# ybubnov/metalchat

Measured on AMD Instinct MI355X. Metric: decode tokens/s (batch=1) + achieved HBM GB/s vs roofline, int4 Llama-3-8B, higher is better.
Workload: dtype bf16

## Files before the change

metalchat_amd/csrc/decoder.cc:

```cpp

#include "decoder_impl.h"

using namespace mcimpl;

mc_decoder::~mc_decoder()
{
    (void)hipSetDevice(dev->ordinal);
    drop_graph();
    for (void* p : allocs) (void)hipFree(p);
    if (blas) blaslt_release(blas);
    if (err_evt) (void)hipEventDestroy(err_evt);
    if (err_host) (void)hipHostFree(err_host);
}

void
mc_decoder::query_occupancy()
{
    if (tb != 2 || occ_fused >= 0) return;
    auto ask = [&](const std::string& name, int block) {
        hipFunction_t f;
        if (fn(name, &f) != MC_OK) return 0;
        int n = 0;
        if (hipModuleOccupancyMaxActiveBlocksPerMultiprocessor(&n, f, block, 0) != hipSuccess) return 0;
        return n;
// ... 111 lines not shown
            P.chain_p = chain % 10;
            return one_launch(block_form::qkv_wo_w13_w, 1, vsh, "mc_attn_qkv_wo_w13_w_bfloat_hd64_k4_q4_f" + std::to_string(P.chain_f) + "p" + std::to_string(P.chain_p));
        }
        if (t) return one_launch(block_form::qkv_wo_w, t, vsh, std::string("mc_attn_qkv_wo_w_bfloat_hd64_k4_q4") + (t > 1 ? "_t" + std::to_string(t) : std::string()));
    }
    if (qkv_wo_in && opt.attn_i8_on && qkv.fmt == MC_WFMT_I8 && wo.fmt == MC_WFMT_I8 && occ_wo_i8 != 0) {
        auto group_ok = [](const linear_w& W) { return W.group == 0 || (W.group >= 16 && (W.group & (W.group - 1)) == 0); };
        const bool built = group_ok(qkv) && group_ok(wo) && qkv.group == wo.group && hd == 128 && wo.in == 4096 && qkv.in == 4096 && KV % 8 == 0 && n_rep <= 16;
        const int t = !built ? 0 : whole_range_tiles({1, 2, 4}, KV, [&](int, int ns, unsigned grid) {
            return deal_ok(pg, ns, 16) && (unsigned)wo.out / 2 <= 8u * grid;
        });
        if (t) return one_launch(block_form::qkv_wo_i8, t, 0, "mc_attn_qkv_wo_i8_bfloat_hd128_k4_q4_t" + std::to_string(t));
    }
    if (qkv_wo_in && i4_shape) {
        auto name = [&] { return "mc_attn_qkv_wo_i4_" + tname + "_hd128_k" + std::to_string(wo.in / 2048) + "_q" + std::to_string(qkv.in / 2048); };
        if (attn_wo_fused(wo) && deal_ok(pg, nsplit, 16) && pg >= 64 && pg <= 512) return one_launch(block_form::qkv_wo_i4, 1, 0, name());
        const int t = !opt.attn_i4_wide_on || occ_wo_i4_wide == 0 || KV % 8 != 0 ? 0 : whole_range_tiles({2, 4}, KV, [&](int, int ns, unsigned grid) {
            return deal_ok(pg, ns, 16) && pg >= 64 && (unsigned)wo.out / 2 <= 16u * grid;
        });
        if (t) return one_launch(block_form::qkv_wo_i4, t, 0, name() + "_t" + std::to_string(t));
    }
    if (!gemma && fused && opt.attn_qkv_on && opt.attn_qkv_only_on && occ_qkv_only != 0 && lin_ok(qkv) && !qkv.lora_cols && qkv_rows_ok && qkv.in == 8192 &&
        cfg.dim == 8192 && hd == 128 && KV % 8 == 0 && (unsigned)(nsplit * KV) <= (unsigned)dev->prop.multiProcessorCount && n_rep <= 16 && pg <= 1024 &&
        deal_ok(pg, nsplit, 24) && pg / nsplit >= 8) {
        P.wo_gemv = true;
        return one_launch(block_form::qkv_only, 1, 0, "mc_attn_qkv_i4_" + tname + "_hd128_q4");
    }
    int qkn_tiles = 0;
    if (gemma && handoffs_ok() && opt.attn_wo_qkn_on && opt.attn_wo_on && opt.attn_qkn_on && hd == 256 && occ_wo_qkn != 0 && lin_ok(wo) && !wo.lora_cols &&
        wo_rows_ok && wo.in == 4096 && n_rep <= 16)
        qkn_tiles = whole_range_tiles({1, 2, 4}, KV, [&](int t_, int, unsigned grid) {
// ... 16 lines not shown
        }
        one_launch(block_form::fused, 1, 0, "mc_attn_fused_" + tname);
        P.fast = handoff_mode_alone();
        P.grid = (unsigned)nsplit * ((P.fast & 2u) ? ((unsigned)KV + 7u) & ~7u : (unsigned)KV);
        return P;
    }
    if (attn_fused_t2()) {
        one_launch(block_form::fused_t2, 2, 0, "mc_attn_fused_t2_" + tname);
        P.fast = opt.handoff_fast ? 1u : 0u;
        return P;
    }
    P.form = block_form::scores_pv;
    P.name = "mc_attn_scores_" + tname;
    P.pv_fold = pv_fold(wo);
    return P;
}

mc_status
mc_decoder::check_handoffs(const step_state& st)
{
    if (!st.err) return MC_OK;
    return report_handoff(st.err);
}

mc_status
mc_decoder::report_handoff(uint32_t code)
{
    handoff_failed();
    char buf[384];
    snprintf(buf, sizeof buf, "decoder: an in-launch hand-off of the decode attention timed out (code 0x%08x): the workgroups of the "
// ... 354 lines not shown
    if (d->first_stage && !d->emb_table) return fail(MC_ERR_RUNTIME, "decoder: tok_embeddings not loaded");
    if (d->last_stage && (!d->output.allocated || !d->final_norm))
        return fail(MC_ERR_RUNTIME, "decoder: output head not loaded");
    if (d->cfg.family == MC_FAMILY_GEMMA3 && !d->pn_ready) {
        for (auto& L : d->layers) {
            if (!L.attention_post_norm || !L.ffn_post_norm) return fail(MC_ERR_RUNTIME, "decoder: post-norm weights are not loaded");
            const postnorm_args a{L.attention_post_norm, d->hidden, d->hidden_b};
            const postnorm_args f{L.ffn_post_norm, d->hidden_b, d->hidden};
            MC_HIP(hipMemcpy(L.pn_attn, &a, sizeof a, hipMemcpyHostToDevice));
            MC_HIP(hipMemcpy(L.pn_ffn, &f, sizeof f, hipMemcpyHostToDevice));
            d->pn_host[L.pn_attn] = a;
            d->pn_host[L.pn_ffn] = f;
        }
        d->pn_ready = true;
    }
    return MC_OK;
}

}

extern "C" {

mc_status
mc_decoder_create(mc_device* dev, mc_library* lib, mc_queue* q, const mc_decoder_config* cfg,
                  mc_decoder** out)
{
    if (!dev || !lib || !q || !cfg || !out)
        return fail(MC_ERR_INVALID_ARGUMENT, "mc_decoder_create: null argument");
    const mc_decoder_config& c = *cfg;
    if (c.n_heads % c.n_kv_heads != 0 || c.n_heads / c.n_kv_heads > 16)
// ... 677 lines not shown
```

metalchat_amd/csrc/decoder_impl.h:

```cpp
#pragma once

#include "backend_impl.h"
#include "decoder_batch.h"
#include "gemv_plan.h"

#include <algorithm>
#include <climits>
#include <cmath>
#include <cstddef>
#include <cstdio>
#include <cstdlib>
#include <cstring>
#include <initializer_list>
#include <map>
#include <memory>
#include <string>
#include <unordered_map>
#include <vector>

struct blaslt_state;

namespace mcimpl {

template <typename... A> inline void
push_all(arg_pack& p, const A&... a)
{
    (p.push(a), ...);
}

struct linear_w {
    int fmt = MC_WFMT_T;
    int out = 0, in = 0, group = 0;
    void* w = nullptr;
    void* scales = nullptr;
    size_t w_bytes = 0, s_bytes = 0;
    size_t row_bytes = 0;
    int ngroups = 1;
    bool allocated = false;
    std::vector<uint8_t> scales_host;
    void* wq2 = nullptr;
    uint64_t wq2_gen = 0;
    void* wd = nullptr;
    uint64_t wd_gen = 0;
    std::unique_ptr<linear_w> lora_a;
    void* lora_b = nullptr;
    std::vector<uint8_t> lora_b_host;
    void* lora_vec = nullptr;
    int lora_rank = 0;
    int lora_cols = 0;
    float lora_scale = 0.0f;
};

struct pick_block {
// ... 177 lines not shown
        return MC_OK;
    }
    float* rope_cos[2] = {nullptr, nullptr};
    float* rope_sin[2] = {nullptr, nullptr};
    int rope_rows = 0;
    int rope_start = 0;
    bool rope_valid = false;
    int last_pos = -1;
    bool want_taps = false;

    hipGraph_t graph = nullptr;
    hipGraphExec_t graph_exec = nullptr;

    std::vector<void*> allocs;
    bool pn_ready = false;
    bool log_on = false;
    std::vector<std::string> launch_log;

    ~mc_decoder();

    mc_status
    alloc(void** p, size_t bytes, bool zero = true)
    {
        hipError_t e = hipMalloc(p, bytes ? bytes : 16);
        if (e != hipSuccess)
            return fail(MC_ERR_ALLOC, std::string("hardware_memory_allocator: failed to allocate ") +
                                          std::to_string(bytes) + " bytes: " + hipGetErrorString(e));
        allocs.push_back(*p);
        if (zero) {
            MC_HIP(hipMemsetAsync(*p, 0, bytes ? bytes : 16, stream));
// ... 50 lines not shown
        void* extra[] = {HIP_LAUNCH_PARAM_BUFFER_POINTER, a.buf.data(), HIP_LAUNCH_PARAM_BUFFER_SIZE,
                         &n, HIP_LAUNCH_PARAM_END};
        mcimpl::launch_range range(name.c_str(), gx, gy, gz, bx, 1, 1);
        if (log_on) launch_log.push_back(name);
        hipError_t e = hipModuleLaunchKernel(f, gx, gy, gz, bx, 1, 1, lds, stream, nullptr, extra);
        if (e != hipSuccess) return hip_fail(e, name.c_str());
        return MC_OK;
    }

    size_t row_bytes(int fmt, int in) const;
    mc_status alloc_linear(linear_w& L, int fmt, int out, int in, int group);
    mc_status upload_rows(linear_w& L, int dst_row0, int dst_stride, int rows, const void* weight, const float* scales, int perm_hd = 0);

    gemv_env genv{};
    static gemv_shape
    shape_of(const linear_w& L) { return {L.fmt, L.out, L.in, L.group, L.lora_cols}; }
    bool
    lin_ok(const linear_w& L) const { return ::lin_ok(shape_of(L), genv); }
    bool
    lin_split_ok(const linear_w& L) const { return ::lin_split_ok(shape_of(L), genv); }
    int
    ling_kib(const linear_w& L) const { return ::ling_kib(shape_of(L), genv); }
    bool
    pv_fold(const linear_w& wo) const
    {
        return opt.pv_fold_on && (lin_ok(wo) || ling_kib(wo)) && !wo.lora_cols && cfg.max_seq_len <= 16384;
    }

    bool
    handoffs_ok() const { return attn_fused_on && attn_psum_g && tb == 2 && n_own <= 254; }
    unsigned
// ... 103 lines not shown
```

metalchat_amd/csrc/decoder_options.h:

```cpp
#pragma once

#include <algorithm>
#include <climits>
#include <cstdlib>

struct decoder_options {
    int gemv_block = 256;
    int gemv_wgs_per_cu = 2;
    bool gemv_block_env = false;
    bool gemv_lin = true;
    bool gemv_ling = true;
    bool i8_ling14 = true;
    bool lin_split = true;
    bool ling_half = true;
    bool lin_k4_on = true;
    int lin_waves = 8;
    bool gemv_full_grid = false;
    int dbg_variant = 0;
    int gemv_m4 = 2;
    int time_gemv_layers = 0;
    bool attn_fused = true;
    unsigned attn_fused_max_wgs_per_cu = 2;
    bool attn_t2_on = true;
    int rearm_after = 256;
    bool handoff_fast = true;
    bool attn_wo_on = true;
    bool attn_wo_k4 = false;
    bool attn_qkv_on = true;
    bool attn_qkv_only_on = false;
    bool attn_i8_on = true;
    bool attn_i4_wide_on = true;
    bool kv_virtual_on = true;
    bool chain_w13_on = true;
    int chain_f = -1;
    bool attn_qkv_qkn_on = true;
// ... 53 lines not shown
    o.gemv_wgs_per_cu = env_int("MC_GEMV_WGS_PER_CU", o.gemv_wgs_per_cu);
    o.gemv_block_env = env_set("MC_GEMV_BLOCK") || env_set("MC_GEMV_WGS_PER_CU");
    if (o.gemv_block % 64 || o.gemv_block < 64 || o.gemv_block > 1024) o.gemv_block = 256;
    if (o.gemv_wgs_per_cu < 1) o.gemv_wgs_per_cu = 2;
    o.gemv_lin = env_flag("MC_GEMV_LIN", o.gemv_lin);
    o.gemv_ling = env_flag("MC_GEMV_LING", o.gemv_ling);
    o.i8_ling14 = env_flag("MC_I8_LING14", o.i8_ling14);
    o.lin_split = env_flag("MC_LIN_SPLIT", o.lin_split);
    o.ling_half = env_flag("MC_LING_HALF", o.ling_half);
    o.lin_k4_on = env_flag("MC_LIN_K4", o.lin_k4_on);
    o.lin_waves = env_int("MC_LIN_WAVES", o.lin_waves, 1, 16);
    o.gemv_full_grid = env_flag("MC_GEMV_FULLGRID", o.gemv_full_grid);
    o.dbg_variant = env_int("MC_GEMV_DBG", o.dbg_variant);
    o.gemv_m4 = env_int("MC_GEMV_M4", o.gemv_m4);
    o.time_gemv_layers = env_int("MC_TIME_GEMV_LAYERS", 0, 0);

    o.attn_fused = env_flag("MC_ATTN_FUSED", o.attn_fused);
    o.attn_fused_max_wgs_per_cu = (unsigned)env_int("MC_ATTN_FUSED_WGS", (int)o.attn_fused_max_wgs_per_cu, 1, 4);
    o.attn_t2_on = env_flag("MC_ATTN_T2", o.attn_t2_on);
    o.rearm_after = env_int("MC_HANDOFF_REARM", o.rearm_after, 0);
    o.handoff_fast = env_flag("MC_HANDOFF_FAST", o.handoff_fast);
    o.attn_wo_on = env_flag("MC_ATTN_WO", o.attn_wo_on);
    o.attn_wo_k4 = env_set("MC_ATTN_WO_K4");
    o.attn_qkv_on = env_flag("MC_ATTN_QKV", o.attn_qkv_on);
    o.attn_qkv_only_on = env_flag("MC_ATTN_QKV_ONLY", o.attn_qkv_only_on);
    o.attn_i8_on = env_flag("MC_ATTN_I8", o.attn_i8_on);
    o.attn_i4_wide_on = env_flag("MC_ATTN_I4_WIDE", o.attn_i4_wide_on);
    o.kv_virtual_on = env_flag("MC_KV_VIRTUAL", o.kv_virtual_on);
    o.chain_w13_on = env_flag("MC_CHAIN_W13", o.chain_w13_on);
    o.chain_f = env_int("MC_CHAIN_F", o.chain_f, 0);
// ... 48 lines not shown
```

metalchat_amd/csrc/gemv_plan.h:

```cpp
#pragma once

#include <algorithm>
#include <cstdint>
#include <string>

#include "../../include/metalchat_hip.h"
#include "decoder_options.h"

struct gemv_shape {
    int fmt, out, in, group, lora_cols;
};
struct gemv_env {
    int tb;
    int qmode;
    unsigned cus;
    unsigned pick_slots;
    const decoder_options* opt;
};
enum class gemv_family { classic, fast, m4, m4d, lin, lin_k4, lin_split, ling };
struct gemv_plan {
    gemv_family family = gemv_family::classic;
    int rows_kib = 0;
    std::string name;
    unsigned wgs = 1, block = 256, lds = 0;
    bool postnorm_by_value = false;
    const char* error = nullptr;
};

inline size_t
gemv_row_bytes(int fmt, int in, int tb)
{
    if (fmt == MC_WFMT_I4) return (size_t)in / 2;
    if (fmt == MC_WFMT_I8) return (size_t)in;
    return (size_t)in * tb;
}
inline bool
gemv_i4_mfma(const gemv_shape& L, const gemv_env& e)
{
    return L.fmt == MC_WFMT_I4 && e.tb == 2 && e.qmode == MC_QMODE_EXACT && e.opt->gemv_m4 && !e.opt->dbg_variant;
// ... 37 lines not shown
}

inline unsigned
gemv_lin_cap(const gemv_env& e)
{
    return e.cus * (e.opt->gemv_block_env ? (unsigned)e.opt->gemv_wgs_per_cu : 1u);
}
inline unsigned
gemv_grid_per_cu(unsigned units, const gemv_env& e, unsigned at_least = 0)
{
    const unsigned waves = (unsigned)e.opt->lin_waves, cap = gemv_lin_cap(e);
    unsigned wgs = std::max((units + waves - 1) / waves, at_least);
    if (wgs > cap) wgs = cap;
    if (wgs > e.cus) wgs = wgs / e.cus * e.cus;
    return wgs;
}

inline gemv_plan
plan_gemv(const gemv_shape& L, const gemv_env& e, int pro, int epi)
{
    const decoder_options& opt = *e.opt;
    const unsigned cus = e.cus;
    gemv_plan P;
    const int nch = gemv_nch(L);
    const bool lin = lin_ok(L, e) && !(pro == 2 && L.lora_cols);
    const int pe_code = pro * 10 + epi;
    const bool lins = !lin && lin_split_ok(L, e) &&
                      (pe_code == 0 || pe_code == 10 || pe_code == 1 || pe_code == 12 || pe_code == 13 || pe_code == 14 || pe_code == 20 || pe_code == 23);
    const int ling = lin || lins || pro == 2 ? 0 : ling_kib(L, e);
    if (pro == 3 && !lin && !ling) {
// ... 14 lines not shown
             : ling ? gemv_family::ling
             : gemv_i4_mfma(L, e) ? (m4d ? gemv_family::m4d : gemv_family::m4)
             : fast ? gemv_family::fast : gemv_family::classic;
    P.rows_kib = lin ? nch : ling;
    P.postnorm_by_value = pro == 2 && (lin || lins);

    const unsigned kpl = L.fmt == MC_WFMT_I4 ? 32 : (L.fmt == MC_WFMT_I8 ? 16 : (e.tb == 2 ? 8 : 4));
    const unsigned chunk = 64 * kpl;
    const unsigned row = (unsigned)((size_t)((L.in + chunk - 1) / chunk) * chunk * e.tb);
    const unsigned lin_block = 64u * (unsigned)opt.lin_waves, parked = (unsigned)opt.lin_waves * 512u;
    const unsigned np = (unsigned)L.out / 2;
    std::string suffix;
    switch (P.family) {
    case gemv_family::lin:
    case gemv_family::lin_k4:
        suffix = "_lin" + std::to_string(nch) + (k4 ? "k4" : "");
        P.wgs = k4 ? cus : gemv_grid_per_cu(np, e);
        P.block = lin_block;
        P.lds = row / 16 * 17 + 128 + parked;
        break;
    case gemv_family::lin_split:
        suffix = "_lin3s";
        P.wgs = gemv_grid_per_cu((unsigned)L.out / 4, e);
        P.block = lin_block;
        P.lds = 3u * chunk * (unsigned)e.tb / 16 * 17 + 128 + parked;
        break;
    case gemv_family::ling: {
        suffix = "_ling" + std::to_string(ling);
        const unsigned waves = (unsigned)opt.lin_waves, cap = gemv_lin_cap(e);
        const bool half = opt.ling_half && (epi == 0 || epi == 1) && !L.lora_cols && 2u * np <= cap * waves && (unsigned)L.out % 2 == 0;
        P.wgs = gemv_grid_per_cu(np, e, half ? std::min(cap, ((unsigned)L.out + waves - 1) / waves) : 0u);
// ... 6 lines not shown
    case gemv_family::fast:
    case gemv_family::classic:
        suffix = P.family == gemv_family::m4d ? "_m4d" : P.family == gemv_family::m4 ? "_m4" : P.family == gemv_family::fast ? "_fast" : "";
        P.wgs = classic_wgs;
        P.block = classic_block;
        P.lds = (P.family == gemv_family::m4d ? row / 16 * 17 : row) + 128;
        break;
    }
    if (L.fmt == MC_WFMT_I4 && e.tb == 2 && opt.dbg_variant && ((pro == 1 && epi == 2) || (pro == 0 && epi == 0)))
        suffix += opt.dbg_variant == 1 ? "_dbgstream" : "_dbgnoload";
    P.name = std::string("mc_gemv_") + (L.fmt == MC_WFMT_I4 ? "i4_" : (L.fmt == MC_WFMT_I8 ? "i8_" : "w_")) + (e.tb == 2 ? "bfloat" : "float") + suffix +
             "_p" + std::to_string(pro) + "_e" + std::to_string(epi);
    if (epi == 5 && P.wgs > e.pick_slots) P.wgs = e.pick_slots;
    return P;
}
```

metalchat_amd/csrc/kernels/attn_block_kernels.hip:

```cpp
#include "gemv.h"

namespace {

using namespace mc;
using namespace mc::gemv;


#ifndef MC_QKV_ROW_DEAL
#define MC_QKV_ROW_DEAL 0
#endif
#ifndef MC_QX_STG_I4
#define MC_QX_STG_I4 1
#endif
#ifndef MC_QX_STG_I8
#define MC_QX_STG_I8 2
#endif
#ifndef MC_QX_STG_W
#define MC_QX_STG_W 0
#endif
template <int HD, int QN, int WB = 0, int STG = (WB == 0 ? MC_QX_STG_I4 : (WB == 1 ? MC_QX_STG_W : MC_QX_STG_I8))>
struct qkv_in_launch {
    static_assert(WB ? QN == 4 : (QN == 2 || QN == 4), "K = 4096 / 8192 int4, 4096 int8, 2048 bfloat; 512 threads");
    static constexpr bool WIDE = WB == 0 && QN == 4;
#ifndef MC_I8_SCORER_WAVES
#define MC_I8_SCORER_WAVES 8
#endif
    static constexpr int SCORER_WAVES = MC_I8_SCORER_WAVES;
    static constexpr bool LDS = true, PIN_V = true, STAGED = STG != 0;
    static constexpr int K_STEPS = WB == 1 ? 1 : (WIDE ? 3 : 2), V_STEP = STG == 2 ? K_STEPS : K_STEPS - 1;
    static constexpr int TL_STRIDE = 16, TL_BASE = 3;
    static constexpr uint32_t KQ = WB == 1 ? 512u * QN : (WB == 2 ? 1024u * QN : 2048u * QN), ROWBQ = 1024u * QN, CHUNK_LDS = 2048 * 2 / 16 * 17, HALF = HD / 2;
    static constexpr uint32_t NPK = KQ / 8;
    static constexpr uint32_t WPK = WB == 1 ? 8u : (WB == 2 ? 16u : 32u);
    static constexpr int PMAXQ = WB == 1 ? 1 : (WIDE ? 3 : 2);
    static constexpr int NXP = WIDE ? 2 : 1;
    typedef const __attribute__((address_space(3))) bf16_t* lds_row;
// ... 586 lines not shown
                    ((gS_p)vt)[((size_t)kv * HD + 2u * j) * max_seq + slot] = va;
                    ((gS_p)vt)[((size_t)kv * HD + 2u * j + 1u) * max_seq + slot] = vb;
                }
            }
        }
        lds_barrier();
        stamp(11);
    }
};

struct gemma_extra {
    const void *post_w, *res_row;
    void* h_out;
    const bf16_t *q_norm, *k_norm;
};
template <int HD, int LNCH, int QN = 0, int WB = 0, int TT = 1, int QKN = 0, int CH = 0>
__device__ __forceinline__ void
attn_wo_body(const bf16_t* __restrict__ q, const bf16_t* __restrict__ kc, const bf16_t* __restrict__ vt, bf16_t* __restrict__ attn_out,
             unsigned long long* psum_g, unsigned long long* slab_g, unsigned long long* row_g, step_state* st, uint32_t n_rep,
             uint32_t KV, uint32_t max_seq, float scale, uint32_t nsplit, uint32_t layer_tag, const void* __restrict__ wo_w,
             const void* __restrict__ wo_s, const bf16_t* res, bf16_t* y, uint32_t out_rows, uint32_t group, uint32_t has_res,
             uint32_t fastpath, unsigned long long* tl,
             const void* __restrict__ qnorm_w = nullptr, const void* __restrict__ qkv_w = nullptr, const void* __restrict__ qkv_s = nullptr,
             const float* fcos = nullptr, const float* fsin = nullptr, unsigned long long* qkv_g = nullptr, float eps = 0.0f, float mu = 0.0f,
             uint32_t kv_shift = 0, gemma_extra gx = gemma_extra(), unsigned long long* hid_g = nullptr)
{
    static_assert(CH == 0 || (QN != 0 && QKN == 0), "a chained phase: behind a llama launch with wq|wk|wv inside");
    constexpr uint32_t K = WB == 1 ? 512u * LNCH : (WB == 2 ? 1024u * LNCH : 2048u * LNCH);
    constexpr uint32_t WPK = WB == 1 ? 8u : (WB == 2 ? 16u : 32u);
    constexpr uint32_t CHUNK_LDS = 2048 * 2 / 16 * 17;
    constexpr uint32_t ROWB = 1024u * LNCH;
    constexpr int QCH = QKN >= 2 ? 3 : QN;
    __shared__ __attribute__((aligned(16))) char xs[(LNCH > QCH ? LNCH : QCH) * (WB == 1 ? 1024u : (WB == 2 ? 2048u : CHUNK_LDS))];
    static_assert(QN == 0 || QKN == 0, "one source of the step's queries");
    __shared__ float qred[(QN || QKN) ? 32 : 1];
    __shared__ __attribute__((aligned(16))) bf16_t qkv_rows[(QN || QKN) ? 18 * HD : 8];
    const uint32_t tid = threadIdx.x, lane = tid & 63, wave = __builtin_amdgcn_readfirstlane(tid >> 6);
    typedef qkv_in_launch<HD, QN ? QN : (WB ? 4 : 2), WB> qx_t;
    qx_t qx;
    if constexpr (QN != 0) {
        typedef typename qx_t::lds_row lds_row;
        qx.q_s = (lds_row)qkv_rows;
        qx.k_s = (lds_row)qkv_rows + n_rep * HD;
        qx.v_s = (lds_row)qkv_rows + (n_rep + 1u) * HD;
        qx.xp = res; qx.normp = qnorm_w; qx.qw = qkv_w; qx.qs = qkv_s; qx.fcos = fcos; qx.fsin = fsin;
        qx.kc = const_cast<bf16_t*>(kc); qx.vt = const_cast<bf16_t*>(vt); qx.qkv_g = qkv_g; qx.st = st; qx.xs = xs; qx.red = qred;
        qx.n_rep = n_rep; qx.KV = KV; qx.max_seq = max_seq; qx.nsplit = nsplit; qx.group = group; qx.layer_tag = layer_tag;
        qx.fastpath = fastpath; qx.eps = eps; qx.mu = mu; qx.tl = tl; qx.kv_shift = kv_shift;
        qx.at_start();
    }
    typedef qkv_qkn_in_launch<(QKN >= 2 ? HD : 256), QKN == 3> qg_t;
    qg_t qg;
    if constexpr (QKN >= 2) {
// ... 202 lines not shown
    stamp(7);
}

}

#define MC_ATTN_WO(NAME, HD, LNCH)                                                                                                        \
    extern "C" __global__ void __launch_bounds__(512)                                                                                    \
    NAME(const bf16_t* q, const bf16_t* kc, const bf16_t* vt, bf16_t* attn_out, unsigned long long* psum_g, unsigned long long* slab_g, \
         unsigned long long* row_g, step_state* st, uint32_t n_rep, uint32_t n_kv, uint32_t max_seq, float scale, uint32_t nsplit,      \
         uint32_t layer_tag, const void* wo_w, const void* wo_s, const bf16_t* res, bf16_t* y, uint32_t out_rows, uint32_t group,       \
         uint32_t has_res, uint32_t fastpath, unsigned long long* tl)                                                                    \
    {                                                                                                                                    \
        attn_wo_body<HD, LNCH>(q, kc, vt, attn_out, psum_g, slab_g, row_g, st, n_rep, n_kv, max_seq, scale, nsplit, layer_tag, wo_w,     \
                               wo_s, res, y, out_rows, group, has_res, fastpath, tl);                                                    \
    }
#define MC_ATTN_QKV_WO(NAME, HD, LNCH, QN, TT)                                                                                            \
    extern "C" __global__ void __launch_bounds__(512)                                                                                    \
    NAME(const bf16_t* kc, const bf16_t* vt, bf16_t* attn_out, unsigned long long* psum_g, unsigned long long* slab_g,                  \
         unsigned long long* row_g, unsigned long long* qkv_g, step_state* st, uint32_t n_rep, uint32_t n_kv, uint32_t max_seq,         \
         float scale, uint32_t nsplit, uint32_t layer_tag, const void* wo_w, const void* wo_s, const bf16_t* x, bf16_t* y,              \
         uint32_t out_rows, uint32_t group, const void* qnorm_w, const void* qkv_w, const void* qkv_s, const float* fcos, const float* fsin, float eps,    \
         float mu, uint32_t fastpath, unsigned long long* tl, uint32_t kv_shift)                                                         \
    {                                                                                                                                    \
        attn_wo_body<HD, LNCH, QN, 0, TT>(nullptr, kc, vt, attn_out, psum_g, slab_g, row_g, st, n_rep, n_kv, max_seq, scale, nsplit,     \
                                          layer_tag, wo_w, wo_s, x, y, out_rows, group, 1u, fastpath, tl, qnorm_w, qkv_w, qkv_s, fcos,   \
                                          fsin, qkv_g, eps, mu, kv_shift);                                                               \
    }
MC_ATTN_QKV_WO(mc_attn_qkv_wo_i4_bfloat_hd128_k2_q2, 128, 2, 2, 1)
MC_ATTN_QKV_WO(mc_attn_qkv_wo_i4_bfloat_hd128_k2_q2_t2, 128, 2, 2, 2)
MC_ATTN_QKV_WO(mc_attn_qkv_wo_i4_bfloat_hd128_k2_q2_t4, 128, 2, 2, 4)
template <int HD, int QN>
__device__ __forceinline__ void
attn_qkv_body(const bf16_t* kc, const bf16_t* vt, bf16_t* attn_out, unsigned long long* psum_g, unsigned long long* slab_g, unsigned long long* qkv_g,
              step_state* st, uint32_t n_rep, uint32_t KV, uint32_t max_seq, float scale, uint32_t nsplit, uint32_t layer_tag, const bf16_t* x,
              uint32_t group, const void* norm_w, const void* qkv_w, const void* qkv_s, const float* fcos, const float* fsin, float eps, float mu,
              uint32_t fastpath, unsigned long long* tl)
{
    constexpr uint32_t CHUNK_LDS = 2048 * 2 / 16 * 17;
    __shared__ __attribute__((aligned(16))) char xs[QN * CHUNK_LDS];
    __shared__ float qred[16];
    __shared__ __attribute__((aligned(16))) bf16_t qkv_rows[18 * HD];
    typedef qkv_in_launch<HD, QN, 0> qx_t;
    typedef typename qx_t::lds_row lds_row;
    qx_t qx;
    qx.q_s = (lds_row)qkv_rows;
// ... 267 lines not shown
```

metalchat_amd/csrc/kernels/decode_kernels.hip:

```cpp
#include "common.h"
#include "handoff.h"
#include <type_traits>

using namespace mc;


__device__ __forceinline__ void
derive_state(step_state* st, int32_t max_seq, int32_t pre_len)
{
    const int32_t post = max_seq - pre_len;
    if (st->pos >= max_seq) {
        st->ring_base = (st->ring_base + 1) % post;
        st->rolled += 1;
        st->write_slot = pre_len + (post - 1 + st->ring_base) % post;
        st->kv_len = max_seq;
    } else {
        const int32_t p = st->pos;
        st->write_slot = p < pre_len ? p : pre_len + (p - pre_len + st->ring_base) % post;
        st->kv_len = p + 1;
    }
    st->rope_row = st->pos - st->rope_start;
    st->epoch += 1;
}

// ... 602 lines not shown
        if (HPP < n_rep + 1u) one_pass(HPP, std::integral_constant<int, 1>{});
        if (2u * HPP < n_rep + 1u) one_pass(2u * HPP, std::integral_constant<int, 2>{});
        for (uint32_t h0 = 3u * HPP; h0 < n_rep + 1u; h0 += HPP) one_pass(h0, std::integral_constant<int, NPRE>{});
        for (uint32_t d = tid; d < (uint32_t)HD; d += NT) {
            const bf16_t v = qkv[(size_t)(H + KV + kv) * HD + d];
            ((lds_row_w)v_s)[d] = v;
            if (writer) vt[((size_t)kv * HD + d) * max_seq + ws] = v;
        }
        lds_barrier();
    }
};
template <typename Q, typename = void>
struct scorer_waves_of { static constexpr int value = 4; };
template <typename Q>
struct scorer_waves_of<Q, std::void_t<decltype(Q::SCORER_WAVES)>> { static constexpr int value = Q::SCORER_WAVES; };
template <int HD, int T, int NW, bool PADKV = false, typename OnChunk, typename BehindScores, typename QSrc = q_from_hbm>
__device__ __forceinline__ void
attn_fused_bf(const bf16_t* __restrict__ q, const bf16_t* __restrict__ kc, const bf16_t* __restrict__ vt,
              unsigned long long* psum_g, unsigned long long* slab_g, step_state* st, uint32_t n_rep, uint32_t KV, uint32_t max_seq,
              float scale, uint32_t nsplit, uint32_t layer_tag, unsigned long long* tl, OnChunk&& on_chunk, BehindScores&& behind_scores,
              uint32_t fastpath, QSrc qsrc = QSrc(), uint32_t kv_shift = 0)
{
    const size_t psum_fast = (size_t)KV * n_rep * nsplit, slab_fast = (size_t)KV * nsplit * n_rep * HD;
    auto stamp = [&](int i) {
        if (tl && threadIdx.x == 0) tl[(size_t)blockIdx.x * QSrc::TL_STRIDE + QSrc::TL_BASE + i] = __builtin_amdgcn_s_memrealtime();
    };
    stamp(0);
    constexpr int KS = HD / 32;
    constexpr int NDB = HD / 16;
    constexpr int NB = NDB >= NW ? NDB / NW : 1;
    constexpr uint32_t PBW = PB * T;
    constexpr int SW = (NW == 8 && T >= 2 && scorer_waves_of<QSrc>::value == 8) ? 8 : 4;
    constexpr int TS = T * 4 / SW;
    constexpr uint32_t PBS = 16u * SW;
    constexpr int ES = PBW + 4;
    __shared__ float wsum[SW][16];
    __shared__ float inv_s[16];
    __shared__ __attribute__((aligned(16))) float ebuf[16 * ES];

    const uint32_t kv_stride = (PADKV && (fastpath & 2u)) ? ((KV + 7u) & ~7u) : KV;
    const uint32_t kv = blockIdx.x % kv_stride, split = blockIdx.x / kv_stride;
    if constexpr (PADKV) {
        if (kv >= KV) return;
    }
    const uint32_t lane = threadIdx.x & 63, wave = threadIdx.x >> 6;
    const uint32_t col = lane & 15, c = lane >> 4;
    const uint32_t p_begin = split * PBW;
    const uint32_t kvc = kv >> kv_shift;
    qsrc.before_tiles();
    uint4 kb[TS][KS];
    const bool scorer = NW == 4 || wave < (uint32_t)SW;
    auto request_k_lds = [&](int t) {
        const size_t live = (size_t)0 - (size_t)(scorer ? 1 : 0);
        const uint32_t pos = p_begin + t * PBS + wave * 16 + col;
        const bf16_t* kbase = kc + ((((size_t)kvc * max_seq + (pos < max_seq ? pos : max_seq - 1)) * HD + c * 8) & live);
#pragma unroll
        for (int ks = 0; ks < KS; ks++) kb[t][ks] = *reinterpret_cast<const uint4*>(kbase + ks * 32);
    };
    if constexpr (QSrc::LDS) {
        if constexpr (!QSrc::STAGED) {
#pragma unroll
            for (int t = 0; t < TS; t++) request_k_lds(t);
        }
    } else if (scorer) {
#pragma unroll
        for (int t = 0; t < TS; t++) {
            const uint32_t pos = p_begin + t * PBS + wave * 16 + col;
            const bf16_t* kbase = kc + ((size_t)kvc * max_seq + (pos < max_seq ? pos : max_seq - 1)) * HD;
#pragma unroll
            for (int ks = 0; ks < KS; ks++) kb[t][ks] = *reinterpret_cast<const uint4*>(kbase + ks * 32 + c * 8);
        }
    }
    uint4 vb[T][NB][2];
    auto request_v = [&] {
#pragma unroll
        for (int t = 0; t < T; t++)
#pragma unroll
            for (int b = 0; b < NB; b++) {
                const uint32_t db = wave + NW * b;
                const bf16_t* vrow = vt + ((size_t)kvc * HD + (db < (uint32_t)NDB ? db : 0u) * 16 + col) * max_seq;
#pragma unroll
                for (int u = 0; u < 2; u++) {
                    const uint32_t p0 = p_begin + t * PB + u * 32 + c * 8;
                    vb[t][b][u] = *reinterpret_cast<const uint4*>(vrow + (p0 + 8 <= max_seq ? p0 : max_seq - 8));
                }
            }
    };
    constexpr bool V_LATE = QSrc::LDS && !QSrc::PIN_V;
    if constexpr (!V_LATE && !QSrc::STAGED) request_v();
    if constexpr (QSrc::LDS && QSrc::STAGED) {
        qsrc.before_scores([&](int step) {
            asm volatile("" ::: "memory");
#pragma unroll
            for (int t = 0; t < TS; t++)
                if (step == (t < QSrc::K_STEPS ? t : QSrc::K_STEPS - 1)) request_k_lds(t);
            if (step == QSrc::V_STEP && !V_LATE) request_v();
            asm volatile("" ::: "memory");
        });
        uint32_t never;
// ... 517 lines not shown
```

metalchat_amd/csrc/kernels/gemv.h:

```cpp
#pragma once
#ifndef MC_ABL_NORM_NOXWAVE
#define MC_ABL_NORM_NOXWAVE 0
#endif

#include "abi.h"
#include "common.h"

#include <type_traits>

namespace mc {
namespace gemv {

enum { WF_T = 0, WF_I8 = 1, WF_I4 = 2 };
enum { Q_EXACT = 0, Q_FAST = 1, Q_DBG_STREAM = 2, Q_DBG_NOLOAD = 3,
       Q_M4 = 5,
       Q_M4D = 6 };
enum { PRO_NONE = 0, PRO_RMSNORM = 1, PRO_POSTNORM = 2, PRO_PARTS = 3 };
constexpr int PARTS_R = 4;

static __device__ __forceinline__ void lds_barrier() { asm volatile("s_waitcnt lgkmcnt(0)\n\ts_barrier" ::: "memory"); }
using abi::postnorm_args;
enum { EPI_STORE = 0, EPI_RESID = 1, EPI_SILU_MUL = 2, EPI_GELU_MUL = 3, EPI_QKV_ROPE = 4, EPI_STORE_PICK = 5 };
using abi::pick_epilogue;
__device__ __forceinline__ unsigned long long
// ... 411 lines not shown
        auto cnt_a = [&](uint32_t i) { return e + sq + (i < sr ? 1u : 0u) + (i < ra ? 1u : 0u); };
        auto cnt_b = [&](uint32_t i) { return e - sq - (i < sr ? 1u : 0u) + (i < rb ? 1u : 0u); };
        const uint32_t a_all = 4u * (e + sq) + sr + ra;
        const uint32_t mine = wave < 4 ? cnt_a(w4) : cnt_b(w4);
        const uint32_t before = wave < 4 ? w4 * (e + sq) + min(w4, sr) + min(w4, ra) : a_all + w4 * (e - sq) - min(w4, sr) + min(w4, rb);
        pb = sb0 + before;
        pe = pb + mine;
    } else {
        const uint32_t nw_total = gridDim.x * nwaves, gw = blockIdx.x * nwaves + wave;
        const uint32_t pq = NP / nw_total, prem = NP - pq * nw_total;
        pb = gw * pq + min(gw, prem);
        pe = pb + pq + (gw < prem ? 1u : 0u);
    }
}

template <int WF, typename T, int QM, int PRO, int EPI, int R, int LNCH = 0, int LTP = 0, int LRING = 0, int LWAVES = 0, int LGEN = 0, int LSPLIT = 0>
__device__ __forceinline__ void
body(const void* __restrict__ wp, const void* __restrict__ sp, const void* __restrict__ xp,
     void* __restrict__ yp, const void* __restrict__ resp, const void* __restrict__ normp,
     uint32_t out_rows, uint32_t in, uint32_t group, float eps, float mu,
     const void* __restrict__ lora_ap, const void* __restrict__ lora_bp, uint32_t lora_rank,
     float lora_scale)
{
    using F = fmt<WF, T>;
    using S = typename T::S;
    constexpr int KPL = F::KPL;
    constexpr uint32_t CHUNK = 64 * KPL;
    constexpr uint32_t CHUNK_BYTES = 64 * 16;
    static_assert(R == 4, "tiles are four rows deep (scale quads, paired epilogues)");

    if (LNCH > 0 || LGEN > 0) {
// ... 696 lines not shown
        auto ltile = [&](uint4 (&dst)[LTP], uint32_t pr, int t, bool live) {
            const uint32_t chunk0 = (uint32_t)(t % SUB) * LTP;
            const uint64_t rb = ((uint64_t)pr * 2 + (uint64_t)(t / SUB)) * rowb_l + (uint64_t)chunk0 * 1024;
            const uint32_t lm = 0u - (uint32_t)live;
            const uint64_t lm64 = ((uint64_t)lm << 32) | lm;
            const char* a = wbase + (rb & lm64);
            const uint32_t lo = lane16 & lm;
#pragma unroll
            for (int p = 0; p < LTP; p++) {
                if (MC_GEMV_LIN_NOLOAD) {
                    dst[p] = make_uint4(lane * 0x01010101u + pr, (lane + pr) * 0x9E3779B9u, lane * 0x85EBCA6Bu + (uint32_t)(t * 0x11111111u),
                                        (p + lane) * 0xC2B2AE35u + pr);
                    continue;
                }
                const u32x4* ap = reinterpret_cast<const u32x4*>(a + p * 1024 + lo);
#ifndef MC_LIN_PLAIN_LOADS
#define MC_LIN_PLAIN_LOADS 0
#endif
                const u32x4 v = MC_LIN_PLAIN_LOADS ? *ap : __builtin_nontemporal_load(ap);
                dst[p] = make_uint4(v.x, v.y, v.z, v.w);
            }
        };
        auto lscales = [&](uint32_t (&q)[LNCH], uint32_t pr, bool live) {
            const uint64_t ub = (((uint64_t)(pr >> 1) * ngroups) * 4 + (pr & 1u) * 2) * 2;
            const uint32_t lm = 0u - (uint32_t)live;
            const char* a = sbase + (ub & (((uint64_t)lm << 32) | lm));
#pragma unroll
            for (int c = 0; c < LNCH; c++) {
                if (MC_GEMV_LIN_NOLOAD) {
                    q[c] = 0x3C003C00u;
                    continue;
                }
                const uint32_t g = group ? ((2048u * (uint32_t)c + 32u * lane) >> glog) : 0u;
                q[c] = *reinterpret_cast<const uint32_t*>(a + ((g * 8u) & lm));
// ... 356 lines not shown
```

metalchat_amd/csrc/kernels/gemv_kernels.hip:

```cpp
#include "gemv.h"
#include "gemv_ksplit.h"

using namespace mc;
using namespace mc::gemv;

#ifndef MC_GEMV_LB
#define MC_GEMV_LB 512
#endif
#define MC_GEMV(NAME, WF, T, QM, PRO, EPI)                                                        \
    extern "C" __global__ void __launch_bounds__(MC_GEMV_LB)                                          \
    NAME(const void* w, const void* scales, const void* x, void* y, const void* res,             \
         const void* norm_w, uint32_t out_rows, uint32_t in, uint32_t group, float eps, float mu, \
         const void* lora_a, const void* lora_b, uint32_t lora_rank, float lora_scale)            \
    {                                                                                             \
        body<WF, T, QM, PRO, EPI, 4>(w, scales, x, y, res, norm_w, out_rows, in, group, eps, mu,  \
                                     lora_a, lora_b, lora_rank, lora_scale);                      \
    }

#ifndef MC_LIN_WAVES
#define MC_LIN_WAVES 8
#endif
#define MC_GEMV_LIN(NAME, PRO, EPI, ...)                                                          \
    extern "C" __global__ void __launch_bounds__(MC_LIN_WAVES ? 64 * MC_LIN_WAVES : MC_GEMV_LB)   \
    NAME(const void* w, const void* scales, const void* x, void* y, const void* res,             \
// ... 56 lines not shown
#endif
#ifndef MC_LIN7_CFG
#define MC_LIN7_CFG 7, 1, 2
#endif
#ifndef MC_LIN12_CFG
#define MC_LIN12_CFG 12, 1, 2
#endif
#ifndef MC_LIN14_CFG
#define MC_LIN14_CFG 14, 1, 2
#endif
MC_GEMV_LIN_SET(mc_gemv_i4_bfloat_lin1, MC_LIN1_CFG)
MC_GEMV_LIN_SET(mc_gemv_i4_bfloat_lin2, MC_LIN2_CFG)
MC_GEMV_LIN_SET(mc_gemv_i4_bfloat_lin4, MC_LIN4_CFG)
MC_GEMV_LIN_SET(mc_gemv_i4_bfloat_lin7, MC_LIN7_CFG)
MC_GEMV_LIN_SET(mc_gemv_i4_bfloat_lin12, MC_LIN12_CFG)
#define MC_GEMV_K4(NAME, NCH, EPI)                                                                \
    extern "C" __global__ void __launch_bounds__(512)                                             \
    NAME(const void* w, const void* scales, const void* x, void* y, const void* res,             \
         const void* norm_w, uint32_t out_rows, uint32_t in, uint32_t group, float eps, float mu, \
         const void* lora_a, const void* lora_b, uint32_t lora_rank, float lora_scale)            \
    {                                                                                             \
        body_ksplit4<NCH, EPI>(w, scales, x, y, res, out_rows, group);                            \
    }
MC_GEMV_K4(mc_gemv_i4_bfloat_lin12k4_p0_e0, 12, 0)
MC_GEMV_K4(mc_gemv_i4_bfloat_lin12k4_p0_e1, 12, 1)
#ifndef MC_LIN3S_RING
#define MC_LIN3S_RING 3
#endif
#define MC_GEMV_LINS(NAME, PRO, EPI)                                                              \
    extern "C" __global__ void __launch_bounds__(64 * MC_LIN_WAVES)                               \
// ... 52 lines not shown
```

Measured before the change: 768.6.

## Plan cache-resident FFN weights and stream KV tiles with non-temporal loads

Adds a planner that picks per-layer w13/w2 weights to keep in the last-level cache, using plain loads through new resident GEMV kernel twins. All other weights keep non-temporal loads. It also adds a non-temporal variant of the fused int4 qkv/wo attention kernel for K/V tile loads, used for layers after the first when the streamed set exceeds the cache size. The aim is to stop streaming data from evicting reusable lines. It risks extra kernel variants, and the resident budget is off by default.

```diff
diff --git a/metalchat_amd/csrc/decoder.cc b/metalchat_amd/csrc/decoder.cc
--- a/metalchat_amd/csrc/decoder.cc
+++ b/metalchat_amd/csrc/decoder.cc
@@ -149,7 +149,8 @@
     }
     if (qkv_wo_in && i4_shape) {
         auto name = [&] { return "mc_attn_qkv_wo_i4_" + tname + "_hd128_k" + std::to_string(wo.in / 2048) + "_q" + std::to_string(qkv.in / 2048); };
-        if (attn_wo_fused(wo) && deal_ok(pg, nsplit, 16) && pg >= 64 && pg <= 512) return one_launch(block_form::qkv_wo_i4, 1, 0, name());
+        const bool nt = kv_nt && tname == "bfloat" && wo.in == 4096 && qkv.in == 4096 && !layers.empty() && &L != &layers[0];
+        if (attn_wo_fused(wo) && deal_ok(pg, nsplit, 16) && pg >= 64 && pg <= 512) return one_launch(block_form::qkv_wo_i4, 1, 0, name() + (nt ? "_nt" : ""));
         const int t = !opt.attn_i4_wide_on || occ_wo_i4_wide == 0 || KV % 8 != 0 ? 0 : whole_range_tiles({2, 4}, KV, [&](int, int ns, unsigned grid) {
             return deal_ok(pg, ns, 16) && pg >= 64 && (unsigned)wo.out / 2 <= 16u * grid;
         });
@@ -196,6 +197,34 @@
     P.name = "mc_attn_scores_" + tname;
     P.pv_fold = pv_fold(wo);
     return P;
+}
+
+void
+mc_decoder::plan_resident_set()
+{
+    resident_planned = true;
+    kv_nt = false;
+    for (layer_w& L : layers) L.w13.resident = L.w2.resident = false;
+    if (!first_stage || !last_stage || layers.empty()) return;
+    const bool gemma = cfg.family == MC_FAMILY_GEMMA3;
+    std::vector<resident_layer> sizes(layers.size());
+    size_t streamed = linear_bytes(output);
+    for (size_t li = 0; li < layers.size(); li++) {
+        layer_w& L = layers[li];
+        streamed += linear_bytes(L.qkv) + linear_bytes(L.wo) + linear_bytes(L.w13) + linear_bytes(L.w2);
+        streamed += 2 * (size_t)cfg.n_kv_heads * cfg.max_seq_len * cfg.head_dim * tb;
+        auto offer = [&](linear_w& W, int pro, int epi) -> size_t {
+            gemv_shape sh = shape_of(W);
+            sh.resident = true;
+            const gemv_plan P = plan_gemv(sh, genv, pro, epi);
+            return !P.error && P.resident ? linear_bytes(W) : (size_t)0;
+        };
+        sizes[li] = resident_layer{{0, 0, gemma ? 0 : offer(L.w13, 1, 2), gemma ? 0 : offer(L.w2, 0, 1)}};
+    }
+    static const std::vector<int> ranks[4] = {{RES_W2, RES_W13}, {RES_W13, RES_W2}, {RES_W2}, {RES_W13}};
+    const auto set = plan_resident(sizes, streamed, (size_t)opt.mall_resident_mb << 20, ranks[opt.mall_rank]);
+    for (const auto& p : set) (p.second == RES_W2 ? layers[p.first].w2 : layers[p.first].w13).resident = true;
+    kv_nt = opt.mall_kv_nt == 2 || (opt.mall_kv_nt == 1 && (streamed > MALL_BYTES || !set.empty()));
 }
 
 mc_status
@@ -580,6 +609,7 @@
         }
         d->pn_ready = true;
     }
+    if (!d->resident_planned) d->plan_resident_set();
     return MC_OK;
 }
 
diff --git a/metalchat_amd/csrc/decoder_impl.h b/metalchat_amd/csrc/decoder_impl.h
--- a/metalchat_amd/csrc/decoder_impl.h
+++ b/metalchat_amd/csrc/decoder_impl.h
@@ -37,6 +37,7 @@
     size_t row_bytes = 0;
     int ngroups = 1;
     bool allocated = false;
+    bool resident = false;
     std::vector<uint8_t> scales_host;
     void* wq2 = nullptr;
     uint64_t wq2_gen = 0;
@@ -244,6 +245,8 @@
 
     std::vector<void*> allocs;
     bool pn_ready = false;
+    bool resident_planned = false, kv_nt = false;
+    void plan_resident_set();
     bool log_on = false;
     std::vector<std::string> launch_log;
 
@@ -324,7 +327,7 @@
 
     gemv_env genv{};
     static gemv_shape
-    shape_of(const linear_w& L) { return {L.fmt, L.out, L.in, L.group, L.lora_cols}; }
+    shape_of(const linear_w& L) { return {L.fmt, L.out, L.in, L.group, L.lora_cols, L.resident}; }
     bool
     lin_ok(const linear_w& L) const { return ::lin_ok(shape_of(L), genv); }
     bool
diff --git a/metalchat_amd/csrc/decoder_options.h b/metalchat_amd/csrc/decoder_options.h
--- a/metalchat_amd/csrc/decoder_options.h
+++ b/metalchat_amd/csrc/decoder_options.h
@@ -19,6 +19,9 @@
     int dbg_variant = 0;
     int gemv_m4 = 2;
     int time_gemv_layers = 0;
+    int mall_resident_mb = 0;
+    int mall_kv_nt = 1;
+    int mall_rank = 0;
     bool attn_fused = true;
     unsigned attn_fused_max_wgs_per_cu = 2;
     bool attn_t2_on = true;
@@ -102,6 +105,9 @@
     o.dbg_variant = env_int("MC_GEMV_DBG", o.dbg_variant);
     o.gemv_m4 = env_int("MC_GEMV_M4", o.gemv_m4);
     o.time_gemv_layers = env_int("MC_TIME_GEMV_LAYERS", 0, 0);
+    o.mall_resident_mb = env_int("MC_MALL_RESIDENT_MB", o.mall_resident_mb, 0, 256);
+    o.mall_kv_nt = env_int("MC_MALL_KV_NT", o.mall_kv_nt, 0, 2);
+    o.mall_rank = env_int("MC_MALL_RANK", o.mall_rank, 0, 3);
 
     o.attn_fused = env_flag("MC_ATTN_FUSED", o.attn_fused);
     o.attn_fused_max_wgs_per_cu = (unsigned)env_int("MC_ATTN_FUSED_WGS", (int)o.attn_fused_max_wgs_per_cu, 1, 4);
diff --git a/metalchat_amd/csrc/gemv_plan.h b/metalchat_amd/csrc/gemv_plan.h
--- a/metalchat_amd/csrc/gemv_plan.h
+++ b/metalchat_amd/csrc/gemv_plan.h
@@ -3,12 +3,15 @@
 #include <algorithm>
 #include <cstdint>
 #include <string>
+#include <utility>
+#include <vector>
 
 #include "../../include/metalchat_hip.h"
 #include "decoder_options.h"
 
 struct gemv_shape {
     int fmt, out, in, group, lora_cols;
+    bool resident = false;
 };
 struct gemv_env {
     int tb;
@@ -23,6 +26,7 @@
     int rows_kib = 0;
     std::string name;
     unsigned wgs = 1, block = 256, lds = 0;
+    bool resident = false;
     bool postnorm_by_value = false;
     const char* error = nullptr;
 };
@@ -90,6 +94,12 @@
     if (wgs > cap) wgs = cap;
     if (wgs > e.cus) wgs = wgs / e.cus * e.cus;
     return wgs;
+}
+
+inline bool
+resident_twin(int nch, int pro, int epi)
+{
+    return (nch == 7 && pro == 0 && epi == 1) || (nch == 2 && pro == 1 && epi == 2);
 }
 
 inline gemv_plan
@@ -134,7 +144,8 @@
     switch (P.family) {
     case gemv_family::lin:
     case gemv_family::lin_k4:
-        suffix = "_lin" + std::to_string(nch) + (k4 ? "k4" : "");
+        P.resident = L.resident && !k4 && opt.lin_waves == 8 && !L.lora_cols && resident_twin(nch, pro, epi);
+        suffix = "_lin" + std::to_string(nch) + (k4 ? "k4" : "") + (P.resident ? "c" : "");
         P.wgs = k4 ? cus : gemv_grid_per_cu(np, e);
         P.block = lin_block;
         P.lds = row / 16 * 17 + 128 + parked;
@@ -171,3 +182,29 @@
     if (epi == 5 && P.wgs > e.pick_slots) P.wgs = e.pick_slots;
     return P;
 }
+
+constexpr size_t MALL_BYTES = (size_t)256 << 20;
+enum resident_kind { RES_QKV = 0, RES_WO = 1, RES_W13 = 2, RES_W2 = 3, RES_KINDS = 4 };
+struct resident_layer {
+    size_t bytes[RES_KINDS];
+};
+inline std::vector<std::pair<int, int>>
+plan_resident(const std::vector<resident_layer>& layers, size_t streamed, size_t budget, const std::vector<int>& ranking)
+{
+    std::vector<std::pair<int, int>> set;
+    if (budget == 0 || streamed <= budget) return set;
+    size_t used = 0;
+    for (const int kind : ranking) {
+        if (kind < 0 || kind >= RES_KINDS) continue;
+        for (size_t li = 1; li < layers.size(); li++) {
+            const size_t b = layers[li].bytes[kind];
+            if (b == 0 || used + b > budget) continue;
+            bool taken = false;
+            for (const auto& p : set) taken = taken || (p.first == (int)li && p.second == kind);
+            if (taken) continue;
+            set.emplace_back((int)li, kind);
+            used += b;
+        }
+    }
+    return set;
+}
diff --git a/metalchat_amd/csrc/kernels/attn_block_kernels.hip b/metalchat_amd/csrc/kernels/attn_block_kernels.hip
--- a/metalchat_amd/csrc/kernels/attn_block_kernels.hip
+++ b/metalchat_amd/csrc/kernels/attn_block_kernels.hip
@@ -18,8 +18,9 @@
 #ifndef MC_QX_STG_W
 #define MC_QX_STG_W 0
 #endif
-template <int HD, int QN, int WB = 0, int STG = (WB == 0 ? MC_QX_STG_I4 : (WB == 1 ? MC_QX_STG_W : MC_QX_STG_I8))>
+template <int HD, int QN, int WB = 0, int STG = (WB == 0 ? MC_QX_STG_I4 : (WB == 1 ? MC_QX_STG_W : MC_QX_STG_I8)), bool KVNT = false>
 struct qkv_in_launch {
+    static constexpr bool KV_NT = KVNT;
     static_assert(WB ? QN == 4 : (QN == 2 || QN == 4), "K = 4096 / 8192 int4, 4096 int8, 2048 bfloat; 512 threads");
     static constexpr bool WIDE = WB == 0 && QN == 4;
 #ifndef MC_I8_SCORER_WAVES
@@ -636,7 +637,7 @@
     void* h_out;
     const bf16_t *q_norm, *k_norm;
 };
-template <int HD, int LNCH, int QN = 0, int WB = 0, int TT = 1, int QKN = 0, int CH = 0>
+template <int HD, int LNCH, int QN = 0, int WB = 0, int TT = 1, int QKN = 0, int CH = 0, int KVNT = 0>
 __device__ __forceinline__ void
 attn_wo_body(const bf16_t* __restrict__ q, const bf16_t* __restrict__ kc, const bf16_t* __restrict__ vt, bf16_t* __restrict__ attn_out,
              unsigned long long* psum_g, unsigned long long* slab_g, unsigned long long* row_g, step_state* st, uint32_t n_rep,
@@ -658,7 +659,8 @@
     __shared__ float qred[(QN || QKN) ? 32 : 1];
     __shared__ __attribute__((aligned(16))) bf16_t qkv_rows[(QN || QKN) ? 18 * HD : 8];
     const uint32_t tid = threadIdx.x, lane = tid & 63, wave = __builtin_amdgcn_readfirstlane(tid >> 6);
-    typedef qkv_in_launch<HD, QN ? QN : (WB ? 4 : 2), WB> qx_t;
+    static_assert(KVNT == 0 || (QN != 0 && WB == 0), "non-temporal K / V tiles: built for the int4 launch with wq|wk|wv inside");
+    typedef qkv_in_launch<HD, QN ? QN : (WB ? 4 : 2), WB, (WB == 0 ? MC_QX_STG_I4 : (WB == 1 ? MC_QX_STG_W : MC_QX_STG_I8)), KVNT != 0> qx_t;
     qx_t qx;
     if constexpr (QN != 0) {
         typedef typename qx_t::lds_row lds_row;
@@ -891,7 +893,7 @@
         attn_wo_body<HD, LNCH>(q, kc, vt, attn_out, psum_g, slab_g, row_g, st, n_rep, n_kv, max_seq, scale, nsplit, layer_tag, wo_w,     \
                                wo_s, res, y, out_rows, group, has_res, fastpath, tl);                                                    \
     }
-#define MC_ATTN_QKV_WO(NAME, HD, LNCH, QN, TT)                                                                                            \
+#define MC_ATTN_QKV_WO(NAME, HD, LNCH, QN, TT, NT)                                                                                          \
     extern "C" __global__ void __launch_bounds__(512)                                                                                    \
     NAME(const bf16_t* kc, const bf16_t* vt, bf16_t* attn_out, unsigned long long* psum_g, unsigned long long* slab_g,                  \
          unsigned long long* row_g, unsigned long long* qkv_g, step_state* st, uint32_t n_rep, uint32_t n_kv, uint32_t max_seq,         \
@@ -899,13 +901,14 @@
          uint32_t out_rows, uint32_t group, const void* qnorm_w, const void* qkv_w, const void* qkv_s, const float* fcos, const float* fsin, float eps,    \
          float mu, uint32_t fastpath, unsigned long long* tl, uint32_t kv_shift)                                                         \
     {                                                                                                                                    \
-        attn_wo_body<HD, LNCH, QN, 0, TT>(nullptr, kc, vt, attn_out, psum_g, slab_g, row_g, st, n_rep, n_kv, max_seq, scale, nsplit,     \
+        attn_wo_body<HD, LNCH, QN, 0, TT, 0, 0, NT>(nullptr, kc, vt, attn_out, psum_g, slab_g, row_g, st, n_rep, n_kv, max_seq, scale, nsplit, \
                                           layer_tag, wo_w, wo_s, x, y, out_rows, group, 1u, fastpath, tl, qnorm_w, qkv_w, qkv_s, fcos,   \
                                           fsin, qkv_g, eps, mu, kv_shift);                                                               \
     }
-MC_ATTN_QKV_WO(mc_attn_qkv_wo_i4_bfloat_hd128_k2_q2, 128, 2, 2, 1)
-MC_ATTN_QKV_WO(mc_attn_qkv_wo_i4_bfloat_hd128_k2_q2_t2, 128, 2, 2, 2)
-MC_ATTN_QKV_WO(mc_attn_qkv_wo_i4_bfloat_hd128_k2_q2_t4, 128, 2, 2, 4)
+MC_ATTN_QKV_WO(mc_attn_qkv_wo_i4_bfloat_hd128_k2_q2, 128, 2, 2, 1, 0)
+MC_ATTN_QKV_WO(mc_attn_qkv_wo_i4_bfloat_hd128_k2_q2_nt, 128, 2, 2, 1, 1)
+MC_ATTN_QKV_WO(mc_attn_qkv_wo_i4_bfloat_hd128_k2_q2_t2, 128, 2, 2, 2, 0)
+MC_ATTN_QKV_WO(mc_attn_qkv_wo_i4_bfloat_hd128_k2_q2_t4, 128, 2, 2, 4, 0)
 template <int HD, int QN>
 __device__ __forceinline__ void
 attn_qkv_body(const bf16_t* kc, const bf16_t* vt, bf16_t* attn_out, unsigned long long* psum_g, unsigned long long* slab_g, unsigned long long* qkv_g,
diff --git a/metalchat_amd/csrc/kernels/decode_kernels.hip b/metalchat_amd/csrc/kernels/decode_kernels.hip
--- a/metalchat_amd/csrc/kernels/decode_kernels.hip
+++ b/metalchat_amd/csrc/kernels/decode_kernels.hip
@@ -640,6 +640,17 @@
 struct scorer_waves_of { static constexpr int value = 4; };
 template <typename Q>
 struct scorer_waves_of<Q, std::void_t<decltype(Q::SCORER_WAVES)>> { static constexpr int value = Q::SCORER_WAVES; };
+template <typename Q, typename = void>
+struct kv_nt_of { static constexpr bool value = false; };
+template <typename Q>
+struct kv_nt_of<Q, std::void_t<decltype(Q::KV_NT)>> { static constexpr bool value = Q::KV_NT; };
+__device__ __forceinline__ uint4
+kv_tile_load_nt(const bf16_t* p)
+{
+    typedef uint32_t kvv4 __attribute__((ext_vector_type(4)));
+    const kvv4 v = __builtin_nontemporal_load(reinterpret_cast<const kvv4*>(p));
+    return make_uint4(v.x, v.y, v.z, v.w);
+}
 template <int HD, int T, int NW, bool PADKV = false, typename OnChunk, typename BehindScores, typename QSrc = q_from_hbm>
 __device__ __forceinline__ void
 attn_fused_bf(const bf16_t* __restrict__ q, const bf16_t* __restrict__ kc, const bf16_t* __restrict__ vt,
@@ -653,6 +664,7 @@
     };
     stamp(0);
     constexpr int KS = HD / 32;
+    constexpr bool KVNT = kv_nt_of<QSrc>::value;
     constexpr int NDB = HD / 16;
     constexpr int NB = NDB >= NW ? NDB / NW : 1;
     constexpr uint32_t PBW = PB * T;
@@ -681,7 +693,10 @@
         const uint32_t pos = p_begin + t * PBS + wave * 16 + col;
         const bf16_t* kbase = kc + ((((size_t)kvc * max_seq + (pos < max_seq ? pos : max_seq - 1)) * HD + c * 8) & live);
 #pragma unroll
-        for (int ks = 0; ks < KS; ks++) kb[t][ks] = *reinterpret_cast<const uint4*>(kbase + ks * 32);
+        for (int ks = 0; ks < KS; ks++) {
+            if constexpr (KVNT) kb[t][ks] = kv_tile_load_nt(kbase + ks * 32);
+            else kb[t][ks] = *reinterpret_cast<const uint4*>(kbase + ks * 32);
+        }
     };
     if constexpr (QSrc::LDS) {
         if constexpr (!QSrc::STAGED) {
@@ -694,7 +709,10 @@
             const uint32_t pos = p_begin + t * PBS + wave * 16 + col;
             const bf16_t* kbase = kc + ((size_t)kvc * max_seq + (pos < max_seq ? pos : max_seq - 1)) * HD;
 #pragma unroll
-            for (int ks = 0; ks < KS; ks++) kb[t][ks] = *reinterpret_cast<const uint4*>(kbase + ks * 32 + c * 8);
+            for (int ks = 0; ks < KS; ks++) {
+                if constexpr (KVNT) kb[t][ks] = kv_tile_load_nt(kbase + ks * 32 + c * 8);
+                else kb[t][ks] = *reinterpret_cast<const uint4*>(kbase + ks * 32 + c * 8);
+            }
         }
     }
     uint4 vb[T][NB][2];
@@ -708,7 +726,8 @@
 #pragma unroll
                 for (int u = 0; u < 2; u++) {
                     const uint32_t p0 = p_begin + t * PB + u * 32 + c * 8;
-                    vb[t][b][u] = *reinterpret_cast<const uint4*>(vrow + (p0 + 8 <= max_seq ? p0 : max_seq - 8));
+                    if constexpr (KVNT) vb[t][b][u] = kv_tile_load_nt(vrow + (p0 + 8 <= max_seq ? p0 : max_seq - 8));
+                    else vb[t][b][u] = *reinterpret_cast<const uint4*>(vrow + (p0 + 8 <= max_seq ? p0 : max_seq - 8));
                 }
             }
     };
diff --git a/metalchat_amd/csrc/kernels/gemv.h b/metalchat_amd/csrc/kernels/gemv.h
--- a/metalchat_amd/csrc/kernels/gemv.h
+++ b/metalchat_amd/csrc/kernels/gemv.h
@@ -449,7 +449,11 @@
     }
 }
 
-template <int WF, typename T, int QM, int PRO, int EPI, int R, int LNCH = 0, int LTP = 0, int LRING = 0, int LWAVES = 0, int LGEN = 0, int LSPLIT = 0>
+#ifndef MC_LIN_PLAIN_LOADS
+#define MC_LIN_PLAIN_LOADS 0
+#endif
+template <int WF, typename T, int QM, int PRO, int EPI, int R, int LNCH = 0, int LTP = 0, int LRING = 0, int LWAVES = 0, int LGEN = 0, int LSPLIT = 0,
+          int LRES = MC_LIN_PLAIN_LOADS>
 __device__ __forceinline__ void
 body(const void* __restrict__ wp, const void* __restrict__ sp, const void* __restrict__ xp,
      void* __restrict__ yp, const void* __restrict__ resp, const void* __restrict__ normp,
@@ -1176,10 +1180,7 @@
                     continue;
                 }
                 const u32x4* ap = reinterpret_cast<const u32x4*>(a + p * 1024 + lo);
-#ifndef MC_LIN_PLAIN_LOADS
-#define MC_LIN_PLAIN_LOADS 0
-#endif
-                const u32x4 v = MC_LIN_PLAIN_LOADS ? *ap : __builtin_nontemporal_load(ap);
+                const u32x4 v = LRES ? *ap : __builtin_nontemporal_load(ap);
                 dst[p] = make_uint4(v.x, v.y, v.z, v.w);
             }
         };
diff --git a/metalchat_amd/csrc/kernels/gemv_kernels.hip b/metalchat_amd/csrc/kernels/gemv_kernels.hip
--- a/metalchat_amd/csrc/kernels/gemv_kernels.hip
+++ b/metalchat_amd/csrc/kernels/gemv_kernels.hip
@@ -94,6 +94,17 @@
 MC_GEMV_LIN_SET(mc_gemv_i4_bfloat_lin4, MC_LIN4_CFG)
 MC_GEMV_LIN_SET(mc_gemv_i4_bfloat_lin7, MC_LIN7_CFG)
 MC_GEMV_LIN_SET(mc_gemv_i4_bfloat_lin12, MC_LIN12_CFG)
+#define MC_GEMV_LIN_RES(NAME, PRO, EPI, ...)                                                      \
+    extern "C" __global__ void __launch_bounds__(MC_LIN_WAVES ? 64 * MC_LIN_WAVES : MC_GEMV_LB)   \
+    NAME(const void* w, const void* scales, const void* x, void* y, const void* res,             \
+         const void* norm_w, uint32_t out_rows, uint32_t in, uint32_t group, float eps, float mu, \
+         const void* lora_a, const void* lora_b, uint32_t lora_rank, float lora_scale)            \
+    {                                                                                             \
+        body<WF_I4, BF, Q_M4D, PRO, EPI, 4, __VA_ARGS__, MC_LIN_WAVES, 0, 0, 1>(                  \
+            w, scales, x, y, res, norm_w, out_rows, in, group, eps, mu, lora_a, lora_b, lora_rank, lora_scale); \
+    }
+MC_GEMV_LIN_RES(mc_gemv_i4_bfloat_lin7c_p0_e1, 0, 1, MC_LIN7_CFG)
+MC_GEMV_LIN_RES(mc_gemv_i4_bfloat_lin2c_p1_e2, 1, 2, MC_LIN2_CFG)
 #define MC_GEMV_K4(NAME, NCH, EPI)                                                                \
     extern "C" __global__ void __launch_bounds__(512)                                             \
     NAME(const void* w, const void* scales, const void* x, void* y, const void* res,             \
```

Measured after the change: 768.5. No clear change (-0.0%).
